# NVIDIA/semantic-segmentation

Hardware: AMD Instinct MI355X
Metric: train images/sec HRNet-OCR-MScale 1024x1024 crop (higher is better)
Workload: dtype fp16; 1 GPU; train_cityscapes_sota: HRNet-OCR-MScale two-scale train step, RMI+BCE loss, crop 1024x1024, batch 1/GPU, SGD, synthetic Cityscapes-shaped batch, random init; global_batch=1, parallelism=dp1, hipgraph=True, optimizer=ssa_sgd_momentum_step, wgrad_side_stream_flush_at=256

## Files before the change

### include/semseg_hip.h

```cpp
#ifndef SEMSEG_HIP_H
#define SEMSEG_HIP_H
#include <stddef.h>
#include <stdint.h>

#ifdef __cplusplus
extern "C" {
#endif

#define SSA_OK 0
#define SSA_EINVAL (-1)
#define SSA_EUNSUPPORTED (-2)

int ssa_version(void);
int ssa_elem_type(void);
const char* ssa_source_sha(void);

int ssa_group_begin(void);
int ssa_group_end(void* stream);
int ssa_group_abort(void);
long ssa_launch_count(int reset);

typedef struct ssa_profile_rec {
  char kernel[120];
  long launches, jobs;
  double total_us, flops, bytes;
} ssa_profile_rec;
int ssa_profile_begin(void);
int ssa_profile_note(double flops, double bytes);
int ssa_profile_end(ssa_profile_rec* out, int max_recs);

typedef struct ssa_conv_desc {
  int B, H, W, Cin;
  int ldx;
  int Ho, Wo, Cout;
  int ldy;
  int KH, KW;
  int stride, pad, dil;
  int transposed;
  int Kpad;
  int out_f32;
  int cfg;
} ssa_conv_desc;

int ssa_conv2d_igemm(const ssa_conv_desc* d, const void* x, const void* w_packed,
                     const float* bias, void* y, void* stream);

int ssa_conv2d_igemm_stats(const ssa_conv_desc* d, const void* x, const void* w_packed,
                           const float* bias, void* y, double* stats, void* stream);

int ssa_conv2d_tile_supported(const ssa_conv_desc* d);
int ssa_conv2d_tile(const ssa_conv_desc* d, const void* x, const void* w_frag,
                    const float* bias, void* y, double* stats, void* stream);
int ssa_bn_stat_replicas(void);
int ssa_conv2d_tile_aux(const ssa_conv_desc* d, const void* x, const void* w_frag,
                        const float* bias, void* y, double* stats, const void* aux, int ldaux,
                        const float* coef, int aux_mode, void* stream);

int ssa_conv2d_tile_p_supported(const ssa_conv_desc* d);
int ssa_conv_tile_strip(int units);
int ssa_conv2d_tile_p(const ssa_conv_desc* d, const void* x, const void* w_frag, const float* bias, void* y,
                      double* stats, const void* aux, int ldaux, const float* coef, int aux_mode, void* stream);

int ssa_conv2d_halo_supported(const ssa_conv_desc* d);
int ssa_conv2d_halo(const ssa_conv_desc* d, const void* x, const void* w_frag,
                    const float* bias, void* y, double* stats, void* stream);

int ssa_conv2d_gemm_wide_supported(const ssa_conv_desc* d);
int ssa_conv2d_gemm_wide(const ssa_conv_desc* d, const void* x, const void* w_frag, const float* bias,
                         void* y, double* stats, void* stream);

int ssa_conv2d_halo_reg_supported(const ssa_conv_desc* d);
int ssa_conv2d_halo_reg(const ssa_conv_desc* d, const void* x, const void* w_frag, const float* bias,
                        void* y, double* stats, void* stream);

int ssa_conv2d_halo5_supported(const ssa_conv_desc* d);
int ssa_conv2d_halo5(const ssa_conv_desc* d, const void* x, const void* w_frag, const float* bias,
                     void* y, double* stats, void* stream);

int ssa_conv2d_igemm_tile(const ssa_conv_desc* d);
int ssa_conv2d_igemm_affine(const ssa_conv_desc* d, const void* x, const void* w_packed, const float* bias, void* y,
                            const float* coef, const void* residual, int ldres, int relu, void* stream);


int ssa_conv2d_dgrad_s2(int B, int H, int W, int Cin, int lddx, int Ho, int Wo, int cout_pad,
                        int lddy, const void* dy, const void* const* w_cls, const int* kpad_cls,
                        void* dx, void* stream);

int ssa_pack_filter(const float* w_oihw, void* w_packed, int Cout, int Cin,
                    int KH, int KW, int cin_pad, int cout_pad, int Kpad,
                    int mode, void* stream);

int ssa_conv2d_wgrad_plan(const ssa_conv_desc* d, int cout_pad, int* nsplit,
                          size_t* ws_bytes);
int ssa_conv2d_wgrad(const ssa_conv_desc* d, const void* x, const void* dy,
                     int lddy, int cout_pad, int nsplit, float* partial,
                     void* stream);
int ssa_conv2d_wgrad_reduce(const float* partial, int nsplit, int cout_pad,
                            int Cout, int Cin_pad, int Cin, int KH, int KW,
                            float* dw_oihw, int accumulate, void* stream);

typedef struct ssa_pack_job {
  const float* w_oihw;
  void* w_packed;
  long elem_begin;
  int Cout, Cin, KH, KW, cin_pad, cout_pad, Kpad, mode, rows;
  int layout;
} ssa_pack_job;
int ssa_pack_filters_batched(const void* jobs_dev, int njobs, int blocks_per_job,
                             void* stream);
int ssa_pack_tile_channels(int KH, int KW);
int ssa_pack_filters_tiled(const void* jobs_dev, const void* tiles_dev, int ntiles,
                           int max_ct_taps, void* stream);

int ssa_conv2d_wgrad_tile_plan(const ssa_conv_desc* d, int cout_pad, int* nsplit,
                               size_t* ws_bytes);
int ssa_conv2d_wgrad_tile(const ssa_conv_desc* d, const void* x, const void* dy,
                          int lddy, int cout_pad, int nsplit, float* partial,
                          void* stream);
int ssa_conv2d_wgrad_tile_geometry(int Cin, int cout_pad, int* parts, int* slots, int* kind);
int ssa_conv2d_wgrad_head_plan(const ssa_conv_desc* d, int cout_pad, int* nsplit,
                               size_t* ws_bytes);
int ssa_conv2d_wgrad_head(const ssa_conv_desc* d, const void* x, const void* dy,
                          int lddy, int cout_pad, int nsplit, float* partial,
                          void* stream);

int ssa_colsum_bf16(const void* x, long P, int C, int ld, float* out,
                    double* scratch2c, void* stream);

int ssa_pad_cast_f32_bf16(const float* x, long P, int C, int ldx, void* y,
                          int Cpad, void* stream);

int ssa_bn_stats(const void* x, long P, int C, int ld, double* sums, int zero_sums,
                 void* stream);
int ssa_bn_apply_train(const void* x, int ldx, const void* residual, int ldr, void* z,
                       int ldz, long P, int C, const double* sums, int nrep, double count,
                       const float* gamma, const float* beta, float* running_mean,
                       float* running_var, long* num_batches_tracked, float momentum,
                       float eps, float* coef, float* pass_stats, int relu,
                       const float* post, long pix_per_img, void* sign_mask, void* stream);
typedef struct ssa_bn_update_job {
  float* running_mean;
  float* running_var;
  long* num_batches_tracked;
  const float* pass_stats[8];
  int C, npass;
  float momentum;
  int pad_;
} ssa_bn_update_job;
int ssa_bn_update_running_batched(const void* jobs_dev, int njobs, int max_channels,
                                  void* stream);
typedef struct ssa_bn_eval_job {
  const float* gamma;
  const float* beta;
  const float* running_mean;
  const float* running_var;
  float* coef;
  int C;
  float eps;
} ssa_bn_eval_job;
int ssa_bn_finalize_eval_batched(const void* jobs_dev, int njobs, int max_channels, void* stream);
int ssa_bn_finalize(const double* sums, double count, int C, const float* gamma,
                    const float* beta, float* running_mean, float* running_var,
                    float momentum, float eps, int use_running, float* scale,
                    float* shift, float* mean, float* invstd, void* stream);
int ssa_bn_apply(const void* x, int ldx, const void* residual, int ldr, void* z,
                 int ldz, long P, int C, const float* scale, const float* shift,
                 int relu, const float* post, long pix_per_img, void* stream);
int ssa_bn_bwd_reduce(const void* x, int ldx, const void* dz, int lddz,
                      const void* z, int ldz, long P, int C, const float* mean,
                      const float* invstd, int relu, const float* post,
                      long pix_per_img, double* sums, int nrep, int zero_sums,
                      const float* mask_scale, const float* mask_shift, const void* sign_mask, void* stream);
int ssa_bn_bwd_apply(const void* x, int ldx, const void* dz, int lddz,
                     const void* z, int ldz, void* dx, int lddx, void* dres,
                     int lddres, long P, int C, const float* gamma,
                     const float* mean, const float* invstd, const double* sums,
                     int nrep, double count, int relu, const float* post,
                     long pix_per_img, float* dgamma, float* dbeta,
                     float param_grad_scale, const float* mask_scale,
                     const float* mask_shift, int accumulate_param_grads, const void* sign_mask, void* stream);
int ssa_add_bn_stats(const void* a, int lda, const void* b, int ldb, void* s, int lds, long P,
                     int C, double* sums, int zero_sums, void* stream);
int ssa_bn_bwd_apply_add(const void* x, int ldx, const void* dz, int lddz,
                         const void* z, int ldz, void* dx, int lddx, void* dres,
                         int lddres, long P, int C, const float* gamma,
                         const float* mean, const float* invstd, const double* sums,
                         int nrep, double count, int relu, const float* post,
                         long pix_per_img, float* dgamma, float* dbeta,
                         float param_grad_scale, const float* mask_scale,
                         const float* mask_shift, int accumulate_param_grads, const void* sign_mask,
                         const void* dadd, int lddadd, void* stream);
int ssa_bn_param_grads(const double* sums, int C, float* dgamma, float* dbeta,
                       void* stream);

int ssa_p2p_buffer_bytes(int world, long slot_doubles, size_t* bytes);
int ssa_p2p_allreduce_f64(double* data, long n, void* const* peers_dev, int rank, int world,
                          unsigned long long* seq_dev, long slot_doubles, void* stream);
int ssa_p2p_timeouts(unsigned* out);
int ssa_p2p_vmm_alloc(size_t bytes, void** ptr, int* fd, size_t* mapped_bytes);
int ssa_p2p_vmm_import(int fd, size_t mapped_bytes, void** ptr);
int ssa_p2p_vmm_unmap(void* ptr, size_t mapped_bytes);

int ssa_sum_act(const void* a, const void* b, const void* c, const void* d,
                void* z, long n, int relu, void* stream);
int ssa_relu_bwd(const void* dz, const void* z, void* g, long n, void* stream);
int ssa_nchw_f32_to_nhwc_bf16(const float* x, void* y, int B, int C, int H, int W,
                              int cpad, void* stream);

int ssa_image_resize_to_nhwc_bf16(const float* x, int B, int C, int Hi, int Wi,
                                  void* y, int Ho, int Wo, int cpad, void* stream);
int ssa_image_resize_to_nhwc(const float* x, int B, int C, int Hi, int Wi,
                             void* y, int Ho, int Wo, int cpad, int align_corners, void* stream);

int ssa_bilinear_fwd(const void* x, int in_dtype, int B, int Hi, int Wi, int C,
                     int ldx, void* y, int out_dtype, int Ho, int Wo, int ldy,
                     void* stream);
int ssa_bilinear_bwd(const void* dy, int dy_dtype, int B, int Ho, int Wo, int C,
                     int lddy, void* dx, int dx_dtype, int Hi, int Wi, int lddx,
                     void* stream);
int ssa_bilinear_bwd_x(const void* dy, int dy_dtype, int B, int Ho, int Wo, int C, int lddy, float* tmp, int Wi,
                       void* stream);
int ssa_bilinear_bwd_y(const float* tmp, int B, int Ho, int Wi, int C, void* dx, int dx_dtype, int Hi, int lddx,
                       void* stream);
// ... 268 lines not shown
```

### semantic-segmentation_amd/csrc/conv_halo_reg.hip

```cpp
#include "conv_epilogue.h"
#include "group.h"
#include "../../include/semseg_hip.h"
#include <stdlib.h>
#include <type_traits>

#ifndef SSA_HREG_DRAIN
#define SSA_HREG_DRAIN (-1)
#endif

namespace {

struct HaloRegArgs {
  const bf16_t* x; const uint4* wfrag; const float* bias; bf16_t* y; double* stats;
  int ldx, Cin, ldy, B, H, W, Cout, nb_total, tiles_x, tiles_y;
};

template <int CK>
struct ConvHaloReg3 {
  typedef HaloRegArgs Args;
  static constexpr int NT = 256;
  static constexpr int WPE = 2;
  static constexpr int NB = 8, TW = 32, TH = 4, BM = TW * TH;
  static constexpr int HW_ = TW + 2, HH_ = TH + 2;
  static constexpr int CP = CK / 8;
  static constexpr int NPIECE = HH_ * HW_ * 8;
  static constexpr int IT = (NPIECE + NT - 1) / NT;
  static constexpr int HWI = (NPIECE + 63) / 64;
  static constexpr int HALO_BYTES = HWI * 1024;
  static constexpr int CST = CK / 16;
  static constexpr int TAPS = 9;
  static constexpr size_t PIPE_BYTES = 2 * (size_t)HALO_BYTES;
  static constexpr int LDC = NB * 32 + 8;
  static constexpr size_t EPI_BYTES = (size_t)BM * LDC * 2;
  static constexpr size_t LDS_BYTES = PIPE_BYTES > EPI_BYTES ? PIPE_BYTES : EPI_BYTES;
  static_assert(CK == 64 || CK == 48, "chunk width");
  static_assert(2 * LDS_BYTES <= 160 * 1024, "two workgroups per CU");

  static __device__ __forceinline__ void run(const Args& a, const int bx, const int by, const int ) {
  const uint4* __restrict__ wfrag = a.wfrag;
  const int ldx = a.ldx, Cin = a.Cin, H = a.H, W = a.W, nb_total = a.nb_total;
  const int tiles_x = a.tiles_x, tiles_y = a.tiles_y;
  SSA_DYN_LDS(unsigned char, smem);

  const int tid = threadIdx.x, lane = tid & 63;
  const int wn = __builtin_amdgcn_readfirstlane(tid >> 6);
  int bid = bx;
  const int tx_i = bid % tiles_x; bid /= tiles_x;
  const int ty_i = bid % tiles_y; bid /= tiles_y;
  const int b = bid;
  const int nb0 = by * NB;
  const int x0 = tx_i * TW, y0 = ty_i * TH;
  const int nchunk = Cin / CK;
  const int csteps = Cin / 16;
  const int ksteps = TAPS * csteps;

  const bf16_t* xb = a.x + (long)b * H * W * ldx;
  unsigned g_off[IT];
  unsigned dma_ok = 0;
#pragma unroll
  for (int i = 0; i < IT; ++i) {
    const int piece = tid + i * NT;
    const int pix = piece >> 3;
    const int hy = pix / HW_, hx = pix - hy * HW_;
    const int q = (piece & 7) ^ ((hx >> 1) & 7);
    const int iy = y0 - 1 + hy, ix = x0 - 1 + hx;
    const bool ok = piece < NPIECE && q < CP && (unsigned)iy < (unsigned)H && (unsigned)ix < (unsigned)W;
    g_off[i] = ok ? (unsigned)((((long)iy * W + ix) * ldx + q * 8) * 2) : 0u;
    dma_ok |= (ok ? 1u : 0u) << i;
  }
  const unsigned lds0 = ssa_lds_addr(smem);
  auto halo_dma = [&](int chunk, int buf) {
    const bf16_t* src = xb + chunk * CK;
#pragma unroll
    for (int i = 0; i < IT; ++i) {
      if ((dma_ok >> i) & 1u) ssa_glds16_untracked_m0(src, g_off[i], lds0 + buf * HALO_BYTES + (i * 4 + wn) * 1024);
    }
  };

  for (int o = tid * 16; o < 2 * HALO_BYTES; o += NT * 16) *reinterpret_cast<uint4*>(smem + o) = make_uint4(0, 0, 0, 0);
  __syncthreads();

  const unsigned char* wq[2];
#pragma unroll
  for (int ni = 0; ni < 2; ++ni) {
    const int nbg = min(nb0 + wn * 2 + ni, nb_total - 1);
    wq[ni] = reinterpret_cast<const unsigned char*>(wfrag + (long)nbg * ksteps * 64);
  }
  const unsigned lane16 = lane * 16;
  constexpr int R = CST == 4 ? 6 : 3;
  constexpr int ROWK = 3 * CST;
  static_assert(ROWK % R == 0 && R <= ROWK, "ring period");
  bf16x8_t bq[R][2];
  auto load_b = [&](const int slot, const int kstep) {
#pragma unroll
    for (int ni = 0; ni < 2; ++ni)
      bq[slot][ni] = *reinterpret_cast<const bf16x8_t*>(wq[ni] + (long)kstep * 1024 + lane16);
  };

  const int a_col = lane & 31;
  const int a_half = (lane >> 5) << 4;
  f32x16_t acc[4][2];
#pragma unroll
  for (int mi = 0; mi < 4; ++mi)
#pragma unroll
    for (int ni = 0; ni < 2; ++ni)
#pragma unroll
      for (int r = 0; r < 16; ++r) acc[mi][ni][r] = 0.f;

  bf16x8_t af[4];
  int a_base[3];
#pragma unroll
  for (int kw = 0; kw < 3; ++kw) {
    const int hx = a_col + kw;
    a_base[kw] = (hx << 7) | ((((hx >> 1) & 7) << 4) ^ a_half);
  }
  auto rd1 = [&](const unsigned char* Hrow, const int kw, const int j, const int mi) {
    af[mi] = *reinterpret_cast<const bf16x8_t*>(Hrow + mi * (HW_ * 128) + (a_base[kw] ^ (j << 5)));
  };

  halo_dma(0, 0);
#pragma unroll
  for (int q = 0; q < R; ++q) load_b(q, (q / CST) * csteps + q % CST);
  ssa_wait_vm_barrier<0, 0>();
  for (int c = 0; c < nchunk; ++c) {
    const unsigned char* Hc = smem + (c & 1) * HALO_BYTES;
    if (c + 1 < nchunk) halo_dma(c + 1, (c + 1) & 1);
#pragma unroll
    for (int mi = 0; mi < 4; ++mi) rd1(Hc, 0, 0, mi);
#pragma nounroll
    for (int kh = 0; kh < 3; ++kh) {
      const unsigned char* Hrow = Hc + kh * (HW_ * 128);
      const int krow = kh * 3 * csteps + c * CST;
      const int krow_n = kh < 2 ? krow + 3 * csteps : min(c + 1, nchunk - 1) * CST;
#pragma unroll
      for (int kw = 0; kw < 3; ++kw) {
#pragma unroll
        for (int j = 0; j < CST; ++j) {
          const int pos = kw * CST + j, slot = pos % R;
#pragma unroll
          for (int mi = 0; mi < 4; ++mi) {
#pragma unroll
            for (int ni = 0; ni < 2; ++ni) acc[mi][ni] = ssa_mfma32(af[mi], bq[slot][ni], acc[mi][ni]);
            if (j + 1 < CST) rd1(Hrow, kw, j + 1, mi);
            else if (kw < 2) rd1(Hrow, kw + 1, 0, mi);
            else rd1(Hrow + HW_ * 128, 0, 0, mi);
          }
          const int pn = pos + R;
          if (pn < ROWK) load_b(slot, krow + (pn / CST) * csteps + pn % CST);
          else load_b(slot, krow_n + ((pn - ROWK) / CST) * csteps + (pn - ROWK) % CST);
#ifndef SSA_EMU
          __builtin_amdgcn_sched_group_barrier(0x008, 2, 0);
          __builtin_amdgcn_sched_group_barrier(0x020, 2, 0);
          __builtin_amdgcn_sched_group_barrier(0x100, 1, 0);
          __builtin_amdgcn_sched_group_barrier(0x008, 2, 0);
          __builtin_amdgcn_sched_group_barrier(0x100, 1, 0);
          __builtin_amdgcn_sched_group_barrier(0x008, 2, 0);
          __builtin_amdgcn_sched_group_barrier(0x100, 1, 0);
          __builtin_amdgcn_sched_group_barrier(0x008, 2, 0);
          __builtin_amdgcn_sched_group_barrier(0x100, 1, 0);
          __builtin_amdgcn_sched_barrier(0);
#endif
        }
      }
    }
    ssa_wait_vm_barrier<SSA_HREG_DRAIN < 0 ? 2 * R : SSA_HREG_DRAIN, 0>();
  }

  const float* __restrict__ bias = a.bias;
  double* __restrict__ stats = a.stats;
  const int ldy = a.ldy, Cout = a.Cout;
  bf16_t* Cs = reinterpret_cast<bf16_t*>(smem);
  double* st = stats ? stats + (long)(bx % ssa::kStatReplicas) * 2 * Cout : nullptr;
  ssa::epi_stage<LDC>(acc, bias, stats != nullptr, 0, wn * 64, nb0 * 32, Cout, Cs, lane,
                      [&](int row) { return y0 + row / TW < H && x0 + row % TW < W; },
                      [&](int, int n, float sv, float qv) {
                        if (n < Cout) {
                          atomicAdd(&st[n], (double)sv);
                          atomicAdd(&st[Cout + n], (double)qv);
                        }
                      });
  __syncthreads();
  bf16_t* yb = a.y + (long)b * H * W * ldy;
  ssa::epi_store_rows<BM, NB * 32, NT>(Cs, nb0 * 32, Cout, tid, [&](int row, bf16_t*& p) {
    const int oy = y0 + row / TW, ox = x0 + row % TW;
    p = yb + ((long)oy * W + ox) * ldy;
    return oy < H && ox < W;
  });
  }
};

bool reg_shape_ok(const ssa_conv_desc* d) {
  if (!d || d->KH != 3 || d->KW != 3 || d->stride != 1 || d->dil != 1 || d->transposed || d->pad != 1) return false;
  if (d->Ho != d->H || d->Wo != d->W || d->out_f32) return false;
  if (d->ldx % 8 || d->Cout % 8 || d->ldy % 8 || ssa::pick_ck(d->Cin) == 0) return false;
  return (long)d->H * d->W * d->ldx * 2 < (1L << 32);
}

}

extern "C" {

int ssa_conv2d_halo_reg_supported(const ssa_conv_desc* d) { return reg_shape_ok(d) ? 1 : 0; }

int ssa_conv2d_halo_reg(const ssa_conv_desc* dp, const void* x, const void* w_frag, const float* bias,
                        void* y, double* stats, void* stream) {
  if (!dp || !x || !w_frag || !y) return SSA_EINVAL;
  if (!reg_shape_ok(dp)) return SSA_EUNSUPPORTED;
  if (!ssa::conv_ptrs_ok(x, y, w_frag)) return SSA_EINVAL;
  const ssa_conv_desc& d = *dp;
  HaloRegArgs a;
  a.x = (const bf16_t*)x; a.wfrag = (const uint4*)w_frag; a.bias = bias; a.y = (bf16_t*)y; a.stats = stats;
  a.ldx = d.ldx; a.Cin = d.Cin; a.ldy = d.ldy; a.B = d.B; a.H = d.H; a.W = d.W; a.Cout = d.Cout;
  a.nb_total = (d.Cout + 31) / 32;
  a.tiles_x = (d.W + 31) / 32; a.tiles_y = (d.H + 3) / 4;
  const int gx = a.tiles_x * a.tiles_y * d.B, gy = (a.nb_total + 7) / 8;
  if (ssa::pick_ck(d.Cin) == 64) {
    typedef ConvHaloReg3<64> K;
    return ssa::submit<K>(a, gx, gy, K::LDS_BYTES, (hipStream_t)stream);
  }
  typedef ConvHaloReg3<48> K;
  return ssa::submit<K>(a, gx, gy, K::LDS_BYTES, (hipStream_t)stream);
}

}
```

### semantic-segmentation_amd/csrc/group.h

```cpp
#pragma once
#include <hip/hip_runtime.h>
#include <string.h>
#include <type_traits>
#include <vector>

namespace ssa {

constexpr int kKernargBudget = 3840;

template <class K, class = void> struct MaxJobs { static constexpr int value = 16; };
template <class K> struct MaxJobs<K, std::void_t<decltype(K::MAXJOBS)>> { static constexpr int value = K::MAXJOBS; };

template <class K>
struct GroupLimits {
  static constexpr int per_job = (int)sizeof(typename K::Args) + 8;
  static constexpr int raw = (kKernargBudget - 16) / per_job;
  static constexpr int cap = MaxJobs<K>::value;
  static constexpr int jobs = raw > cap ? cap : (raw < 1 ? 1 : raw);
};

template <class K>
struct GroupTable {
  int n, pad_;
  int end[GroupLimits<K>::jobs];
  int gx[GroupLimits<K>::jobs];
  typename K::Args a[GroupLimits<K>::jobs];
};

template <class K, class = void> struct WavesPerEu { static constexpr int value = 1; };
template <class K> struct WavesPerEu<K, std::void_t<decltype(K::WPE)>> { static constexpr int value = K::WPE; };

template <class K>
__global__ __launch_bounds__(K::NT, WavesPerEu<K>::value) void k_single(const typename K::Args a) {
  K::run(a, blockIdx.x, blockIdx.y, gridDim.x);
}

template <class K>
__global__ __launch_bounds__(K::NT, WavesPerEu<K>::value) void k_grouped(const GroupTable<K> t) {
  constexpr int J = GroupLimits<K>::jobs;
  const int bx = (int)blockIdx.x;
  int j = 0;
#pragma unroll
  for (int i = 0; i + 1 < J; ++i) j += bx >= t.end[i] ? 1 : 0;
  const int prev = t.end[j > 0 ? j - 1 : 0];
  const int gx = t.gx[j];
  const int v = bx - (j > 0 ? prev : 0);
  int vx = v, vy = 0;
  if (v >= gx) { vy = v / gx; vx = v - vy * gx; }
  K::run(t.a[j], vx, vy, gx);
}

struct Bucket {
  const void* key;
  int (*flush)(Bucket&, hipStream_t);
  std::vector<unsigned char> args;
  std::vector<int> gx, gy;
  std::vector<double> flops, bytes;
  size_t lds;
};

bool profiling();
void profile_take_note(double* flops, double* bytes);
void* profile_open(const char* kernel, hipStream_t s);
void profile_close(void* h, hipStream_t s, int jobs, double flops, double bytes);

template <class K>
const char* kernel_name() { return __PRETTY_FUNCTION__; }

struct GroupState {
  int depth = 0;
  int error = 0;
  std::vector<Bucket> buckets;
};

GroupState& group_state();
void count_launches(int n);


constexpr int kMaxDevices = 16;
struct LdsLimit { size_t set_to[kMaxDevices] = {}; };

inline int raise_lds_limit(const void* fn, size_t lds, size_t threshold, LdsLimit* lim) {
  if (lds <= threshold) return 0;
  int dev = 0;
  if (hipGetDevice(&dev) != hipSuccess || dev < 0 || dev >= kMaxDevices) dev = 0;
  if (lds > lim->set_to[dev]) {
    hipError_t e = hipFuncSetAttribute(fn, hipFuncAttributeMaxDynamicSharedMemorySize, (int)lds);
    if (e != hipSuccess) return (int)e;
    lim->set_to[dev] = lds;
  }
  return 0;
}

template <class K>
int ensure_lds(const void* fn, size_t lds, LdsLimit* lim) {
  return raise_lds_limit(fn, lds, 64 * 1024, lim);
}

template <class K>
int flush_bucket(Bucket& b, hipStream_t s) {
  typedef typename K::Args Args;
  constexpr int J = GroupLimits<K>::jobs;
  static LdsLimit lds_single, lds_grouped;
  const int n = (int)b.gx.size();
  for (int j0 = 0; j0 < n; j0 += J) {
    const int cnt = n - j0 < J ? n - j0 : J;
    if (cnt == 1) {
      Args a;
      memcpy(&a, b.args.data() + (size_t)j0 * sizeof(Args), sizeof(Args));
      if (int e = ensure_lds<K>((const void*)k_single<K>, b.lds, &lds_single)) return e;
      void* ph = profiling() ? profile_open(kernel_name<K>(), s) : nullptr;
      hipLaunchKernelGGL(k_single<K>, dim3(b.gx[j0], b.gy[j0]), dim3(K::NT), b.lds, s, a);
      if (ph) profile_close(ph, s, 1, b.flops[j0], b.bytes[j0]);
    } else {
      GroupTable<K> t;
      memset(&t, 0, sizeof(t));
      t.n = cnt;
      int total = 0;
      for (int i = 0; i < cnt; ++i) {
        total += b.gx[j0 + i] * b.gy[j0 + i];
        t.end[i] = total;
        t.gx[i] = b.gx[j0 + i];
        memcpy(&t.a[i], b.args.data() + (size_t)(j0 + i) * sizeof(Args), sizeof(Args));
      }
      for (int i = cnt - 1; i < J; ++i) t.end[i] = 0x7fffffff;
      if (int e = ensure_lds<K>((const void*)k_grouped<K>, b.lds, &lds_grouped)) return e;
      void* ph = profiling() ? profile_open(kernel_name<K>(), s) : nullptr;
      hipLaunchKernelGGL(k_grouped<K>, dim3(total), dim3(K::NT), b.lds, s, t);
      if (ph) {
        double fl = 0, by = 0;
        for (int i = 0; i < cnt; ++i) { fl += b.flops[j0 + i]; by += b.bytes[j0 + i]; }
        profile_close(ph, s, cnt, fl, by);
      }
    }
    count_launches(1);
    hipError_t e = hipGetLastError();
    if (e != hipSuccess) return (int)e;
  }
  return 0;
}

template <class K>
int submit(const typename K::Args& a, int gx, int gy, size_t lds, hipStream_t s) {
  typedef typename K::Args Args;
  static_assert(sizeof(GroupTable<K>) <= kKernargBudget + 64, "job table exceeds the kernel-argument budget");
  if (gx <= 0 || gy <= 0) return -1;
  GroupState& g = group_state();
  double note_f = 0, note_b = 0;
  const bool prof = profiling();
  if (prof) profile_take_note(&note_f, &note_b);
  if (g.depth == 0) {
    static LdsLimit lds_single;
    if (int e = ensure_lds<K>((const void*)k_single<K>, lds, &lds_single)) return e;
    void* ph = prof ? profile_open(kernel_name<K>(), s) : nullptr;
    hipLaunchKernelGGL(k_single<K>, dim3(gx, gy), dim3(K::NT), lds, s, a);
    if (ph) profile_close(ph, s, 1, note_f, note_b);
    count_launches(1);
    hipError_t e = hipGetLastError();
    return e == hipSuccess ? 0 : (int)e;
  }
  const void* key = (const void*)k_grouped<K>;
  Bucket* b = nullptr;
  for (Bucket& c : g.buckets)
    if (c.key == key) { b = &c; break; }
  if (!b) {
    g.buckets.push_back(Bucket{key, &flush_bucket<K>, {}, {}, {}, {}, {}, 0});
    b = &g.buckets.back();
  }
  const size_t off = b->args.size();
  b->args.resize(off + sizeof(Args));
  memcpy(b->args.data() + off, &a, sizeof(Args));
  b->gx.push_back(gx);
  b->gy.push_back(gy);
  b->flops.push_back(note_f);
  b->bytes.push_back(note_b);
  if (lds > b->lds) b->lds = lds;
  return 0;
}

}
```

### semantic-segmentation_amd/semseg_amd/_lib.py

```python
import ctypes
import os
from ctypes import c_int, c_long, c_float, c_double, c_void_p, c_size_t, c_uint64, POINTER

_HERE = os.path.dirname(os.path.abspath(__file__))
ACT = os.environ.get("SSA_ACT_DTYPE", "bf16").lower()
if ACT in ("f16", "float16", "half"):
    ACT = "fp16"
if ACT not in ("bf16", "fp16"):
    raise RuntimeError("SSA_ACT_DTYPE must be bf16 or fp16, not %r" % ACT)
LIB_PATH = os.path.normpath(os.path.join(_HERE, "..", "lib", "libsemseg_hip.so" if ACT == "bf16" else "libsemseg_hip_f16.so"))
CSRC = os.path.normpath(os.path.join(_HERE, "..", "csrc"))

_LIB = None


def source_sha():
    import glob
    import hashlib
    files = sorted(glob.glob(os.path.join(CSRC, "*.hip"))) + sorted(glob.glob(os.path.join(CSRC, "*.h"))) + [
        os.path.normpath(os.path.join(_HERE, "..", "..", "include", "semseg_hip.h"))]
    if not files or not all(os.path.exists(f) for f in files):
        return None
    h = hashlib.sha256()
    for f in files:
        with open(f, "rb") as fh:
            h.update(fh.read())
    return h.hexdigest()[:16]


class PackJob(ctypes.Structure):
    _fields_ = [("w", c_void_p), ("out", c_void_p), ("elem_begin", c_long)] + [(n, c_int) for n in (
        "Cout", "Cin", "KH", "KW", "cin_pad", "cout_pad", "Kpad", "mode", "rows", "layout")]


class BnEvalJob(ctypes.Structure):
    _fields_ = [("gamma", c_void_p), ("beta", c_void_p), ("running_mean", c_void_p), ("running_var", c_void_p),
                ("coef", c_void_p), ("C", c_int), ("eps", c_float)]


class BnUpdateJob(ctypes.Structure):
    _fields_ = [("running_mean", c_void_p), ("running_var", c_void_p), ("num_batches_tracked", c_void_p),
                ("pass_stats", c_void_p * 8), ("C", c_int), ("npass", c_int), ("momentum", c_float),
                ("pad_", c_int)]


class ProfileRec(ctypes.Structure):
    _fields_ = [("kernel", ctypes.c_char * 120), ("launches", c_long), ("jobs", c_long),
                ("total_us", c_double), ("flops", c_double), ("bytes", c_double)]


class ConvDesc(ctypes.Structure):
    _fields_ = [(n, c_int) for n in (
        "B", "H", "W", "Cin", "ldx", "Ho", "Wo", "Cout", "ldy", "KH", "KW",
        "stride", "pad", "dil", "transposed", "Kpad", "out_f32", "cfg")]


class DwConvDesc(ctypes.Structure):
    _fields_ = [(n, c_int) for n in ("B", "H", "W", "C", "ldx", "Ho", "Wo", "ldy", "stride", "dil")]


class GConvDesc(ctypes.Structure):
    _fields_ = [(n, c_int) for n in ("B", "H", "W", "C", "G", "ldx", "Ho", "Wo", "ldy", "stride", "dil")]


class JitterProgram(ctypes.Structure):
    _fields_ = [("n_ops", c_int), ("op", c_int * 4), ("factor", c_float * 3), ("hue_byte", c_int)]


class GblurTaps(ctypes.Structure):
    _fields_ = [("radius", c_int), ("w", c_double * 6)]


class RandaugProgram(ctypes.Structure):
    _fields_ = [("n_ops", c_int), ("op", c_int * 8), ("value", c_double * 8), ("matrix", (c_double * 6) * 8)]


_P = c_void_p
_SIGS = {
    "ssa_version": ([], c_int),
    "ssa_elem_type": ([], c_int),
    "ssa_source_sha": ([], ctypes.c_char_p),
    "ssa_group_begin": ([], c_int),
    "ssa_group_end": ([_P], c_int),
    "ssa_group_abort": ([], c_int),
    "ssa_launch_count": ([c_int], c_long),
    "ssa_profile_begin": ([], c_int),
    "ssa_profile_note": ([c_double, c_double], c_int),
    "ssa_profile_end": ([POINTER(ProfileRec), c_int], c_int),
    "ssa_conv2d_igemm": ([POINTER(ConvDesc), _P, _P, _P, _P, _P], c_int),
    "ssa_conv2d_igemm_stats": ([POINTER(ConvDesc), _P, _P, _P, _P, _P, _P], c_int),
    "ssa_conv2d_igemm_tile": ([POINTER(ConvDesc)], c_int),
    "ssa_conv2d_tile_supported": ([POINTER(ConvDesc)], c_int),
    "ssa_conv2d_tile": ([POINTER(ConvDesc), _P, _P, _P, _P, _P, _P], c_int),
    "ssa_conv2d_tile_aux": ([POINTER(ConvDesc), _P, _P, _P, _P, _P, _P, c_int, _P, c_int, _P], c_int),
    "ssa_bn_stat_replicas": ([], c_int),
    "ssa_conv2d_tile_p_supported": ([POINTER(ConvDesc)], c_int),
    "ssa_conv_tile_strip": ([c_int], c_int),
    "ssa_conv2d_tile_p": ([POINTER(ConvDesc), _P, _P, _P, _P, _P, _P, c_int, _P, c_int, _P], c_int),
    "ssa_conv2d_halo_supported": ([POINTER(ConvDesc)], c_int),
    "ssa_conv2d_halo": ([POINTER(ConvDesc), _P, _P, _P, _P, _P, _P], c_int),
    "ssa_conv2d_gemm_wide_supported": ([POINTER(ConvDesc)], c_int),
    "ssa_conv2d_gemm_wide": ([POINTER(ConvDesc), _P, _P, _P, _P, _P, _P], c_int),
    "ssa_conv2d_halo_reg_supported": ([POINTER(ConvDesc)], c_int),
    "ssa_conv2d_halo_reg": ([POINTER(ConvDesc), _P, _P, _P, _P, _P, _P], c_int),
    "ssa_conv2d_halo5_supported": ([POINTER(ConvDesc)], c_int),
    "ssa_conv2d_halo5": ([POINTER(ConvDesc), _P, _P, _P, _P, _P, _P], c_int),
    "ssa_pack_filter": ([_P, _P] + [c_int] * 8 + [_P], c_int),
    "ssa_conv2d_wgrad_plan": ([POINTER(ConvDesc), c_int, POINTER(c_int), POINTER(c_size_t)], c_int),
    "ssa_conv2d_wgrad": ([POINTER(ConvDesc), _P, _P, c_int, c_int, c_int, _P, _P], c_int),
    "ssa_conv2d_wgrad_tile_plan": ([POINTER(ConvDesc), c_int, POINTER(c_int), POINTER(c_size_t)], c_int),
    "ssa_conv2d_wgrad_tile": ([POINTER(ConvDesc), _P, _P, c_int, c_int, c_int, _P, _P], c_int),
    "ssa_conv2d_wgrad_tile_geometry": ([c_int, c_int, POINTER(c_int), POINTER(c_int), POINTER(c_int)], c_int),
    "ssa_conv2d_wgrad_head_plan": ([POINTER(ConvDesc), c_int, POINTER(c_int), POINTER(c_size_t)], c_int),
    "ssa_conv2d_wgrad_head": ([POINTER(ConvDesc), _P, _P, c_int, c_int, c_int, _P, _P], c_int),
    "ssa_conv2d_wgrad_reduce": ([_P] + [c_int] * 7 + [_P, c_int, _P], c_int),
    "ssa_colsum_bf16": ([_P, c_long, c_int, c_int, _P, _P, _P], c_int),
    "ssa_pad_cast_f32_bf16": ([_P, c_long, c_int, c_int, _P, c_int, _P], c_int),
    "ssa_bn_stats": ([_P, c_long, c_int, c_int, _P, c_int, _P], c_int),
    "ssa_bn_apply_train": ([_P, c_int, _P, c_int, _P, c_int, c_long, c_int, _P, c_int, c_double, _P, _P, _P, _P,
                            _P, c_float, c_float, _P, _P, c_int, _P, c_long, _P, _P], c_int),
    "ssa_bn_update_running_batched": ([_P, c_int, c_int, _P], c_int),
    "ssa_pack_filters_batched": ([_P, c_int, c_int, _P], c_int),
    "ssa_pack_tile_channels": ([c_int, c_int], c_int),
    "ssa_conv2d_dgrad_s2": ([c_int] * 9 + [_P, _P, _P, _P, _P], c_int),
    "ssa_pack_filters_tiled": ([_P, _P, c_int, c_int, _P], c_int),
    "ssa_conv2d_igemm_affine": ([POINTER(ConvDesc), _P, _P, _P, _P, _P, _P, c_int, c_int, _P], c_int),
    "ssa_bn_finalize_eval_batched": ([_P, c_int, c_int, _P], c_int),
    "ssa_bn_finalize": ([_P, c_double, c_int, _P, _P, _P, _P, c_float, c_float, c_int,
                         _P, _P, _P, _P, _P], c_int),
    "ssa_bn_apply": ([_P, c_int, _P, c_int, _P, c_int, c_long, c_int, _P, _P, c_int, _P,
                      c_long, _P], c_int),
    "ssa_bn_bwd_reduce": ([_P, c_int, _P, c_int, _P, c_int, c_long, c_int, _P, _P, c_int, _P,
                           c_long, _P, c_int, c_int, _P, _P, _P, _P], c_int),
    "ssa_bn_bwd_apply": ([_P, c_int, _P, c_int, _P, c_int, _P, c_int, _P, c_int, c_long, c_int,
                          _P, _P, _P, _P, c_int, c_double, c_int, _P, c_long, _P, _P, c_float, _P, _P, c_int, _P, _P], c_int),
    "ssa_add_bn_stats": ([_P, c_int, _P, c_int, _P, c_int, c_long, c_int, _P, c_int, _P], c_int),
    "ssa_bn_bwd_apply_add": ([_P, c_int, _P, c_int, _P, c_int, _P, c_int, _P, c_int, c_long, c_int,
                              _P, _P, _P, _P, c_int, c_double, c_int, _P, c_long, _P, _P, c_float, _P, _P, c_int, _P,
                              _P, c_int, _P], c_int),
    "ssa_bn_param_grads": ([_P, c_int, _P, _P, _P], c_int),
    "ssa_p2p_buffer_bytes": ([c_int, c_long, POINTER(c_size_t)], c_int),
    "ssa_p2p_allreduce_f64": ([_P, c_long, _P, c_int, c_int, _P, c_long, _P], c_int),
    "ssa_p2p_timeouts": ([_P], c_int),
    "ssa_p2p_vmm_alloc": ([c_size_t, POINTER(c_void_p), POINTER(c_int), POINTER(c_size_t)], c_int),
    "ssa_p2p_vmm_import": ([c_int, c_size_t, POINTER(c_void_p)], c_int),
    "ssa_p2p_vmm_unmap": ([_P, c_size_t], c_int),
    "ssa_sum_act": ([_P, _P, _P, _P, _P, c_long, c_int, _P], c_int),
    "ssa_relu_bwd": ([_P, _P, _P, c_long, _P], c_int),
    "ssa_nchw_f32_to_nhwc_bf16": ([_P, _P, c_int, c_int, c_int, c_int, c_int, _P], c_int),
    "ssa_image_resize_to_nhwc_bf16": ([_P, c_int, c_int, c_int, c_int, _P, c_int, c_int, c_int, _P], c_int),
    "ssa_bilinear_fwd": ([_P, c_int, c_int, c_int, c_int, c_int, c_int, _P, c_int, c_int, c_int,
                          c_int, _P], c_int),
    "ssa_bilinear_bwd": ([_P, c_int, c_int, c_int, c_int, c_int, c_int, _P, c_int, c_int, c_int,
                          c_int, _P], c_int),
    "ssa_bilinear_bwd_x": ([_P, c_int, c_int, c_int, c_int, c_int, c_int, _P, c_int, _P], c_int),
    "ssa_bilinear_bwd_y": ([_P, c_int, c_int, c_int, c_int, _P, c_int, c_int, c_int, _P], c_int),
    "ssa_image_resize_to_nhwc": ([_P, c_int, c_int, c_int, c_int, _P, c_int, c_int, c_int, c_int, _P], c_int),
    "ssa_resize_bilinear_fwd": ([_P, c_int, c_int, c_int, c_int, c_int, c_int, _P, c_int, c_int, c_int,
                                 c_int, c_int, _P], c_int),
    "ssa_resize_bilinear_bwd": ([_P, c_int, c_int, c_int, c_int, c_int, c_int, _P, c_int, c_int, c_int,
                                 c_int, c_int, _P], c_int),
    "ssa_resize_bilinear_bwd_x": ([_P, c_int, c_int, c_int, c_int, c_int, c_int, _P, c_int, c_int, _P], c_int),
    "ssa_resize_bilinear_bwd_y": ([_P, c_int, c_int, c_int, c_int, _P, c_int, c_int, c_int, c_int, _P], c_int),
    "ssa_maxpool3x3s2_fwd": ([_P, c_int, c_int, c_int, c_int, c_int, _P, _P, c_int, c_int, _P], c_int),
    "ssa_maxpool3x3s2_bwd": ([_P, _P, c_int, c_int, c_int, c_int, _P, c_int, c_int, _P], c_int),
    "ssa_maxpool3x3s2c_fwd": ([_P, c_int, c_int, c_int, c_int, c_int, _P, _P, c_int, c_int, _P], c_int),
    "ssa_maxpool3x3s2c_bwd": ([_P, _P, c_int, c_int, c_int, c_int, _P, c_int, c_int, _P], c_int),
    "ssa_gconv3x3": ([POINTER(GConvDesc), _P, _P, _P, _P, _P], c_int),
    "ssa_gconv3x3_bwd_plan": ([POINTER(GConvDesc), POINTER(c_size_t)], c_int),
    "ssa_gconv3x3_bwd": ([POINTER(GConvDesc), _P, _P, c_int, _P, _P, c_int, _P, c_int, _P, _P], c_int),
    "ssa_se_plan": ([c_int, c_long, c_int, c_int, POINTER(c_size_t)], c_int),
    "ssa_se_squeeze_gate": ([_P, c_int, c_int, c_long, c_int, c_int, _P, _P, _P, _P, _P, _P, _P, _P, _P], c_int),
    "ssa_se_apply": ([_P, c_int, _P, c_int, _P, _P, c_int, c_int, c_long, c_int, c_int, _P], c_int),
    "ssa_se_bwd_reduce": ([_P, c_int, _P, c_int, _P, c_int, c_int, c_long, c_int, c_int, _P, _P, _P], c_int),
    "ssa_se_gate_bwd": ([_P, _P, _P, _P, _P, _P, c_int, c_long, c_int, c_int, _P, _P, _P, _P, _P, c_int, _P, _P], c_int),
    "ssa_se_apply_bwd": ([_P, c_int, _P, c_int, _P, _P, c_int, c_long, c_int, c_int, _P, c_int, _P, c_int, _P], c_int),
    "ssa_dwconv3x3": ([POINTER(DwConvDesc), _P, _P, _P, _P, _P, c_int, _P], c_int),
    "ssa_dwconv3x3_bwd_plan": ([POINTER(DwConvDesc), POINTER(c_size_t)], c_int),
    "ssa_dwconv3x3_bwd": ([POINTER(DwConvDesc), _P, _P, c_int, _P, _P, c_int, _P, c_int, _P, _P], c_int),
    "ssa_global_avg_pool_fwd": ([_P, c_int, c_int, c_long, c_int, _P, _P], c_int),
    "ssa_global_avg_pool_bwd": ([_P, c_int, c_long, c_int, _P, _P], c_int),
    "ssa_resize_nearest_u8": ([_P, c_int, c_int, c_int, _P, c_int, c_int, _P, _P, _P], c_int),
    "ssa_softmax_hw_stats": ([_P, c_int, c_long, c_int, _P, _P], c_int),
    "ssa_softmax_hw_probs": ([_P, c_int, c_long, c_int, _P, _P, c_int, _P], c_int),
    "ssa_rowdot_f32": ([_P, _P, c_int, c_int, _P, _P], c_int),
    "ssa_softmax_hw_bwd": ([_P, c_int, c_long, c_int, _P, _P, c_int, _P, _P, c_int, c_int, _P], c_int),
    "ssa_softmax_lastdim_fwd": ([_P, c_int, c_long, c_int, c_float, _P, c_int, _P], c_int),
    "ssa_softmax_lastdim_bwd": ([_P, c_int, c_long, c_int, c_float, _P, c_int, _P, c_int, _P], c_int),
    "ssa_pack_matrix": ([_P, c_int, c_int, c_int, c_int, c_int, _P, c_int, c_int, _P], c_int),
    "ssa_ocr_attn_supported": ([c_int, c_int], c_int),
    "ssa_ocr_attn_fwd": ([_P, c_int, _P, _P, c_long, c_int, c_int, c_float, _P, c_int, _P], c_int),
    "ssa_ocr_attn_bwd": ([_P, c_int, _P, _P, _P, c_int, c_long, c_int, c_int, c_float, _P, c_int, _P, _P, _P], c_int),
    "ssa_sigmoid_fwd": ([_P, _P, c_long, _P], c_int),
    "ssa_sigmoid_bwd": ([_P, _P, _P, c_long, _P], c_int),
    "ssa_bcast_mul_fwd": ([_P, _P, _P, c_long, c_int, _P], c_int),
    "ssa_bcast_mul_bwd": ([_P, _P, _P, _P, _P, c_long, c_int, _P], c_int),
    "ssa_attn_blend_fwd": ([_P, _P, _P, _P, c_long, c_int, _P], c_int),
    "ssa_attn_blend_bwd": ([_P, _P, _P, _P, _P, c_long, c_int, c_int, _P], c_int),
    "ssa_ce_fwd": ([_P, c_int, _P, c_long, c_int, c_int, _P, _P, _P], c_int),
    "ssa_bce_fwd": ([_P, c_int, _P, c_long, c_int, _P, _P, _P], c_int),
    "ssa_loss_finalize": ([_P, c_double, _P, _P], c_int),
    "ssa_bce_bwd": ([_P, c_int, _P, c_long, c_int, _P, c_double, _P, c_double, _P, _P], c_int),
    "ssa_scale_grad": ([_P, c_long, _P, c_double, _P, c_double, _P], c_int),
    "ssa_scale_grad_to": ([_P, _P, c_long, _P, c_double, _P, c_double, _P], c_int),
    "ssa_rmi_pool": ([_P, c_int, _P, c_int, c_int, c_int, c_int, _P, _P, c_int, c_int, _P], c_int),
    "ssa_rmi_gram": ([_P, _P, c_int, c_int, c_int, _P, _P], c_int),
    "ssa_rmi_solve": ([_P, c_int, c_int, c_int, _P, _P, _P], c_int),
    "ssa_rmi_finalize": ([_P, c_int, c_int, _P, _P], c_int),
    "ssa_rmi_bwd_pooled": ([_P, _P, _P, c_int, c_int, c_int, _P, _P], c_int),
    "ssa_rmi_bwd_logits": ([_P, c_int, _P, c_int, c_int, c_int, c_int, _P, c_int, c_int, _P,
                            c_double, _P, c_int, _P], c_int),
    "ssa_rmi_bwd_logits_bce": ([_P, c_int, _P, c_int, c_int, c_int, c_int, _P, c_int, c_int, _P, c_double, _P, c_double, _P,
                                c_double, _P, _P], c_int),
    "ssa_relax_mask_labels": ([_P, c_int, c_int, c_int, c_int, c_int, c_int, c_int, c_uint64, c_uint64, _P, _P, _P], c_int),
    "ssa_relax_mask_multihot": ([_P, c_int, c_int, c_int, c_int, _P, _P, _P], c_int),
    "ssa_relax_multihot": ([_P, c_int, c_int, c_int, c_int, _P, _P], c_int),
    "ssa_relax_weights": ([_P, c_int, c_int, c_double, c_int, _P, _P, _P], c_int),
    "ssa_relax_nll_fwd": ([_P, c_int, _P, _P, c_int, c_int, c_int, c_int, _P, _P], c_int),
    "ssa_relax_nll_finalize": ([_P, _P, c_int, c_int, c_int, c_int, _P, _P], c_int),
    "ssa_relax_nll_bwd": ([_P, c_int, _P, _P, _P, c_int, c_int, c_int, c_int, _P, _P, _P], c_int),
    "ssa_image_u8_crop_flip_normalize": ([_P, c_int, c_int, c_int, c_int, c_int, c_int, c_int, _P, _P, _P, c_int, _P],
                                         c_int),
    "ssa_resample_u8": ([_P, c_int, c_int, c_int, c_int, _P, c_int, _P, _P, c_int, _P], c_int),
    "ssa_label_u8_crop_flip": ([_P, c_int, c_int, c_int, c_int, c_int, c_int, c_int, _P, _P], c_int),
    "ssa_jitter_luma_sum": ([_P, c_int, c_int, c_int, c_int, c_int, c_int, POINTER(JitterProgram), _P, _P], c_int),
    "ssa_jitter_apply_u8": ([_P, c_int, c_int, c_int, c_int, c_int, c_int, c_int, POINTER(JitterProgram), _P, _P, _P],
                            c_int),
    "ssa_jitter_crop_flip_normalize": ([_P, c_int, c_int, c_int, c_int, c_int, c_int, c_int, POINTER(JitterProgram), _P,
                                        _P, _P, _P, c_int, _P], c_int),
    "ssa_gblur_u8": ([_P, c_int, c_int, c_int, c_int, c_int, c_int, c_int, POINTER(JitterProgram), _P, POINTER(GblurTaps),
                      _P, _P, _P], c_int),
    "ssa_gblur_crop_flip_normalize": ([_P, c_int, c_int, c_int, c_int, c_int, c_int, c_int, POINTER(JitterProgram), _P,
                                       POINTER(GblurTaps), _P, _P, _P, _P, c_int, _P], c_int),
    "ssa_randaug_u8": ([_P, _P, c_int, c_int, c_int, c_int, c_int, c_int, c_int, POINTER(RandaugProgram), c_int, _P, _P, _P,
                        _P, _P, _P], c_int),
    "ssa_class_centroids_u8": ([_P, c_int, c_int, c_int, c_int, c_int, c_int, _P, _P, _P, _P], c_int),
    "ssa_pad_u8": ([_P, c_int, c_int, c_int, c_int, c_int, c_int, c_int, ctypes.c_char_p, _P, _P], c_int),
    "ssa_autolabel_u8": ([_P, _P, _P, c_int, c_int, c_int, c_int, c_int, c_int, ctypes.c_char_p, c_int, c_int, c_int, c_int,
                          c_int, c_int, c_int, c_int, _P, _P, _P, c_int, _P], c_int),
    "ssa_confusion_matrix": ([_P, c_int, _P, c_long, c_int, _P, _P, _P], c_int),
    "ssa_eval_tail": ([_P, _P, c_int, c_int, c_int, c_int, c_int, c_int, _P, c_int, c_float, c_float, _P, _P, _P, _P, _P,
                       _P, _P], c_int),
    "ssa_dump_tail": ([_P, c_long, POINTER(c_float), POINTER(c_float), _P, _P, _P, _P, _P, _P, c_float, c_int, c_int,
                       _P, _P, _P, _P, _P, _P, _P, _P], c_int),
    "ssa_mask_u8": ([_P, c_long, _P, _P], c_int),
    "ssa_sgd_momentum_step": ([_P, _P, _P, _P, c_int, c_float, _P, c_float, c_float, c_int, _P, _P], c_int),
    "ssa_amp_check_grads": ([_P, _P, c_int, _P, _P], c_int),
    "ssa_amp_update": ([_P, c_int, c_float, c_float, c_float, c_float, _P], c_int),
    "ssa_amp_update_counted": ([_P, _P, c_int, c_float, c_float, c_float, c_float, _P], c_int),
    "ssa_adam_advance": ([_P, c_int, c_int, c_double, c_double, _P, _P], c_int),
    "ssa_adam_step": ([_P, _P, _P, _P, _P, _P, _P, c_int, c_int, c_float, _P, c_double, c_double, c_float, c_float,
                       _P, _P], c_int),
    "ssa_ewise_f32": ([c_int, _P, _P, _P, c_long, _P], c_int),
    "ssa_ewise_bwd_f32": ([c_int, _P, _P, _P, _P, _P, c_long, _P], c_int),
    "ssa_axpy_f32": ([_P, c_float, _P, c_long, c_int, _P], c_int),
# ... 50 lines not shown
```

Before: 53.82 images/s.

## Split tail-wave tiles into half-height tiles in halo_reg conv to balance waves

Adds a host-side plan step that counts total workgroups against the CU count and, when the last wave is only partly filled and a cost model favours it, splits the trailing tiles into two half-height (2-row) tiles. The kernel body is templated on the row count so half tiles use fewer MFMA accumulators and a smaller halo, and the epilogue stats are merged across the two accumulator halves. The goal is to shorten the tail-wave imbalance (wave quantization) in 3x3 conv launches. The risks are extra halo-load overhead for the split tiles and a more complex epilogue stats path.

```diff
diff --git a/include/semseg_hip.h b/include/semseg_hip.h
--- a/include/semseg_hip.h
+++ b/include/semseg_hip.h
@@ -69,6 +69,7 @@
 int ssa_conv2d_gemm_wide(const ssa_conv_desc* d, const void* x, const void* w_frag, const float* bias,
                          void* y, double* stats, void* stream);
 
+int ssa_conv_halo_reg_slots(int slots);
 int ssa_conv2d_halo_reg_supported(const ssa_conv_desc* d);
 int ssa_conv2d_halo_reg(const ssa_conv_desc* d, const void* x, const void* w_frag, const float* bias,
                         void* y, double* stats, void* stream);
diff --git a/semantic-segmentation_amd/csrc/conv_halo_reg.hip b/semantic-segmentation_amd/csrc/conv_halo_reg.hip
--- a/semantic-segmentation_amd/csrc/conv_halo_reg.hip
+++ b/semantic-segmentation_amd/csrc/conv_halo_reg.hip
@@ -13,20 +13,58 @@
 struct HaloRegArgs {
   const bf16_t* x; const uint4* wfrag; const float* bias; bf16_t* y; double* stats;
   int ldx, Cin, ldy, B, H, W, Cout, nb_total, tiles_x, tiles_y;
+  int split_from, ntiles;
 };
+
+constexpr double kHalfTileCost = 0.58;
+int g_slots = -1;
+
+int device_slots() {
+  static int cached[ssa::kMaxDevices] = {};
+  int dev = 0;
+  if (hipGetDevice(&dev) != hipSuccess || dev < 0 || dev >= ssa::kMaxDevices) dev = 0;
+  if (cached[dev] == 0) {
+    int cus = 0;
+    if (hipDeviceGetAttribute(&cus, hipDeviceAttributeMultiprocessorCount, dev) != hipSuccess || cus <= 0) return 0;
+    cached[dev] = cus;
+  }
+  return cached[dev];
+}
+
+int split_count(long N, int S) {
+  if (S <= 0 || N <= 0) return 0;
+  const long r = N % S;
+  if (r == 0) return 0;
+  const long short_rounds = (2 * r + S - 1) / S;
+  return short_rounds * kHalfTileCost < 1.0 ? (int)r : 0;
+}
+
+void plan_jobs(HaloRegArgs* a, int* gx, int* gy, int n) {
+  long N = 0;
+  for (int j = 0; j < n; ++j) N += (long)gx[j] * gy[j];
+  int left = split_count(N, g_slots < 0 ? device_slots() : g_slots);
+  for (int j = n - 1; j >= 0 && left > 0; --j) {
+    const int nj = gx[j] * gy[j];
+    const int take = left < nj ? left : nj;
+    a[j].split_from = nj - take;
+    gx[j] = nj + take;
+    gy[j] = 1;
+    left -= take;
+  }
+}
 
 template <int CK>
 struct ConvHaloReg3 {
   typedef HaloRegArgs Args;
+  static void plan(Args* a, int* gx, int* gy, int n) { plan_jobs(a, gx, gy, n); }
   static constexpr int NT = 256;
   static constexpr int WPE = 2;
   static constexpr int NB = 8, TW = 32, TH = 4, BM = TW * TH;
   static constexpr int HW_ = TW + 2, HH_ = TH + 2;
   static constexpr int CP = CK / 8;
-  static constexpr int NPIECE = HH_ * HW_ * 8;
-  static constexpr int IT = (NPIECE + NT - 1) / NT;
-  static constexpr int HWI = (NPIECE + 63) / 64;
-  static constexpr int HALO_BYTES = HWI * 1024;
+  static constexpr int npiece(int MR) { return (MR + 2) * HW_ * 8; }
+  static constexpr int halo_bytes(int MR) { return (npiece(MR) + 63) / 64 * 1024; }
+  static constexpr int HALO_BYTES = halo_bytes(TH);
   static constexpr int CST = CK / 16;
   static constexpr int TAPS = 9;
   static constexpr size_t PIPE_BYTES = 2 * (size_t)HALO_BYTES;
@@ -37,6 +75,20 @@
   static_assert(2 * LDS_BYTES <= 160 * 1024, "two workgroups per CU");
 
   static __device__ __forceinline__ void run(const Args& a, const int bx, const int by, const int ) {
+    if (a.split_from < 0) { body<TH>(a, bx, by, 0); return; }
+    const int h = bx - a.split_from;
+    const int u = h < 0 ? bx : a.split_from + (h >> 1);
+    const int slice = u / a.ntiles, tile = u - slice * a.ntiles;
+    if (h < 0) body<TH>(a, tile, slice, 0);
+    else body<TH / 2>(a, tile, slice, (h & 1) * (TH / 2));
+  }
+
+  template <int MR>
+  static __device__ __forceinline__ void body(const Args& a, const int bx, const int by, const int yoff) {
+  constexpr int NPIECE = npiece(MR);
+  constexpr int IT = (NPIECE + NT - 1) / NT;
+  constexpr int HALO_BYTES = halo_bytes(MR);
+  constexpr int BM = MR * TW;
   const uint4* __restrict__ wfrag = a.wfrag;
   const int ldx = a.ldx, Cin = a.Cin, H = a.H, W = a.W, nb_total = a.nb_total;
   const int tiles_x = a.tiles_x, tiles_y = a.tiles_y;
@@ -49,7 +101,9 @@
   const int ty_i = bid % tiles_y; bid /= tiles_y;
   const int b = bid;
   const int nb0 = by * NB;
-  const int x0 = tx_i * TW, y0 = ty_i * TH;
+  const int x0 = tx_i * TW, y0 = ty_i * TH + yoff;
+  if constexpr (MR != TH)
+    if (y0 >= a.H) return;
   const int nchunk = Cin / CK;
   const int csteps = Cin / 16;
   const int ksteps = TAPS * csteps;
@@ -99,15 +153,15 @@
 
   const int a_col = lane & 31;
   const int a_half = (lane >> 5) << 4;
-  f32x16_t acc[4][2];
-#pragma unroll
-  for (int mi = 0; mi < 4; ++mi)
+  f32x16_t acc[MR / 2][2][2];
+#pragma unroll
+  for (int mi = 0; mi < MR; ++mi)
 #pragma unroll
     for (int ni = 0; ni < 2; ++ni)
 #pragma unroll
-      for (int r = 0; r < 16; ++r) acc[mi][ni][r] = 0.f;
-
-  bf16x8_t af[4];
+      for (int r = 0; r < 16; ++r) acc[mi >> 1][mi & 1][ni][r] = 0.f;
+
+  bf16x8_t af[MR];
   int a_base[3];
 #pragma unroll
   for (int kw = 0; kw < 3; ++kw) {
@@ -126,7 +180,7 @@
     const unsigned char* Hc = smem + (c & 1) * HALO_BYTES;
     if (c + 1 < nchunk) halo_dma(c + 1, (c + 1) & 1);
 #pragma unroll
-    for (int mi = 0; mi < 4; ++mi) rd1(Hc, 0, 0, mi);
+    for (int mi = 0; mi < MR; ++mi) rd1(Hc, 0, 0, mi);
 #pragma nounroll
     for (int kh = 0; kh < 3; ++kh) {
       const unsigned char* Hrow = Hc + kh * (HW_ * 128);
@@ -138,9 +192,9 @@
         for (int j = 0; j < CST; ++j) {
           const int pos = kw * CST + j, slot = pos % R;
 #pragma unroll
-          for (int mi = 0; mi < 4; ++mi) {
-#pragma unroll
-            for (int ni = 0; ni < 2; ++ni) acc[mi][ni] = ssa_mfma32(af[mi], bq[slot][ni], acc[mi][ni]);
+          for (int mi = 0; mi < MR; ++mi) {
+#pragma unroll
+            for (int ni = 0; ni < 2; ++ni) acc[mi >> 1][mi & 1][ni] = ssa_mfma32(af[mi], bq[slot][ni], acc[mi >> 1][mi & 1][ni]);
             if (j + 1 < CST) rd1(Hrow, kw, j + 1, mi);
             else if (kw < 2) rd1(Hrow, kw + 1, 0, mi);
             else rd1(Hrow + HW_ * 128, 0, 0, mi);
@@ -154,10 +208,12 @@
           __builtin_amdgcn_sched_group_barrier(0x100, 1, 0);
           __builtin_amdgcn_sched_group_barrier(0x008, 2, 0);
           __builtin_amdgcn_sched_group_barrier(0x100, 1, 0);
-          __builtin_amdgcn_sched_group_barrier(0x008, 2, 0);
-          __builtin_amdgcn_sched_group_barrier(0x100, 1, 0);
-          __builtin_amdgcn_sched_group_barrier(0x008, 2, 0);
-          __builtin_amdgcn_sched_group_barrier(0x100, 1, 0);
+          if constexpr (MR == 4) {
+            __builtin_amdgcn_sched_group_barrier(0x008, 2, 0);
+            __builtin_amdgcn_sched_group_barrier(0x100, 1, 0);
+            __builtin_amdgcn_sched_group_barrier(0x008, 2, 0);
+            __builtin_amdgcn_sched_group_barrier(0x100, 1, 0);
+          }
           __builtin_amdgcn_sched_barrier(0);
 #endif
         }
@@ -171,12 +227,21 @@
   const int ldy = a.ldy, Cout = a.Cout;
   bf16_t* Cs = reinterpret_cast<bf16_t*>(smem);
   double* st = stats ? stats + (long)(bx % ssa::kStatReplicas) * 2 * Cout : nullptr;
-  ssa::epi_stage<LDC>(acc, bias, stats != nullptr, 0, wn * 64, nb0 * 32, Cout, Cs, lane,
-                      [&](int row) { return y0 + row / TW < H && x0 + row % TW < W; },
-                      [&](int, int n, float sv, float qv) {
+  auto valid = [&](int row) { return y0 + row / TW < H && x0 + row % TW < W; };
+  double ups[2] = {0., 0.}, upq[2] = {0., 0.};
+  if constexpr (MR == TH)
+    ssa::epi_stage<LDC>(acc[0], bias, stats != nullptr, 0, wn * 64, nb0 * 32, Cout, Cs, lane, valid,
+                        [&](int col, int, float sv, float qv) {
+                          const bool second = col - wn * 64 >= 32;
+                          if (second) { ups[1] = (double)sv; upq[1] = (double)qv; }
+                          else { ups[0] = (double)sv; upq[0] = (double)qv; }
+                        });
+  ssa::epi_stage<LDC>(acc[MR / 2 - 1], bias, stats != nullptr, BM - 2 * TW, wn * 64, nb0 * 32, Cout, Cs, lane, valid,
+                      [&](int col, int n, float sv, float qv) {
                         if (n < Cout) {
-                          atomicAdd(&st[n], (double)sv);
-                          atomicAdd(&st[Cout + n], (double)qv);
+                          const bool second = col - wn * 64 >= 32;
+                          atomicAdd(&st[n], (second ? ups[1] : ups[0]) + (double)sv);
+                          atomicAdd(&st[Cout + n], (second ? upq[1] : upq[0]) + (double)qv);
                         }
                       });
   __syncthreads();
@@ -201,6 +266,12 @@
 extern "C" {
 
 int ssa_conv2d_halo_reg_supported(const ssa_conv_desc* d) { return reg_shape_ok(d) ? 1 : 0; }
+
+int ssa_conv_halo_reg_slots(int slots) {
+  const int prev = g_slots;
+  g_slots = slots < 0 ? -1 : slots;
+  return prev;
+}
 
 int ssa_conv2d_halo_reg(const ssa_conv_desc* dp, const void* x, const void* w_frag, const float* bias,
                         void* y, double* stats, void* stream) {
@@ -214,6 +285,7 @@
   a.nb_total = (d.Cout + 31) / 32;
   a.tiles_x = (d.W + 31) / 32; a.tiles_y = (d.H + 3) / 4;
   const int gx = a.tiles_x * a.tiles_y * d.B, gy = (a.nb_total + 7) / 8;
+  a.split_from = -1; a.ntiles = gx;
   if (ssa::pick_ck(d.Cin) == 64) {
     typedef ConvHaloReg3<64> K;
     return ssa::submit<K>(a, gx, gy, K::LDS_BYTES, (hipStream_t)stream);
diff --git a/semantic-segmentation_amd/csrc/group.h b/semantic-segmentation_amd/csrc/group.h
--- a/semantic-segmentation_amd/csrc/group.h
+++ b/semantic-segmentation_amd/csrc/group.h
@@ -29,6 +29,10 @@
 
 template <class K, class = void> struct WavesPerEu { static constexpr int value = 1; };
 template <class K> struct WavesPerEu<K, std::void_t<decltype(K::WPE)>> { static constexpr int value = K::WPE; };
+
+template <class K, class = void> struct HasPlan : std::false_type {};
+template <class K>
+struct HasPlan<K, std::void_t<decltype(K::plan((typename K::Args*)nullptr, (int*)nullptr, (int*)nullptr, 0))>> : std::true_type {};
 
 template <class K>
 __global__ __launch_bounds__(K::NT, WavesPerEu<K>::value) void k_single(const typename K::Args a) {
@@ -105,6 +109,12 @@
   const int n = (int)b.gx.size();
   for (int j0 = 0; j0 < n; j0 += J) {
     const int cnt = n - j0 < J ? n - j0 : J;
+    if constexpr (HasPlan<K>::value) {
+      Args pa[J];
+      memcpy(pa, b.args.data() + (size_t)j0 * sizeof(Args), (size_t)cnt * sizeof(Args));
+      K::plan(pa, b.gx.data() + j0, b.gy.data() + j0, cnt);
+      memcpy(b.args.data() + (size_t)j0 * sizeof(Args), pa, (size_t)cnt * sizeof(Args));
+    }
     if (cnt == 1) {
       Args a;
       memcpy(&a, b.args.data() + (size_t)j0 * sizeof(Args), sizeof(Args));
@@ -152,8 +162,15 @@
   if (g.depth == 0) {
     static LdsLimit lds_single;
     if (int e = ensure_lds<K>((const void*)k_single<K>, lds, &lds_single)) return e;
+    const Args* la = &a;
+    [[maybe_unused]] Args planned;
+    if constexpr (HasPlan<K>::value) {
+      planned = a;
+      K::plan(&planned, &gx, &gy, 1);
+      la = &planned;
+    }
     void* ph = prof ? profile_open(kernel_name<K>(), s) : nullptr;
-    hipLaunchKernelGGL(k_single<K>, dim3(gx, gy), dim3(K::NT), lds, s, a);
+    hipLaunchKernelGGL(k_single<K>, dim3(gx, gy), dim3(K::NT), lds, s, *la);
     if (ph) profile_close(ph, s, 1, note_f, note_b);
     count_launches(1);
     hipError_t e = hipGetLastError();
diff --git a/semantic-segmentation_amd/semseg_amd/_lib.py b/semantic-segmentation_amd/semseg_amd/_lib.py
--- a/semantic-segmentation_amd/semseg_amd/_lib.py
+++ b/semantic-segmentation_amd/semseg_amd/_lib.py
@@ -101,6 +101,7 @@
     "ssa_conv2d_halo": ([POINTER(ConvDesc), _P, _P, _P, _P, _P, _P], c_int),
     "ssa_conv2d_gemm_wide_supported": ([POINTER(ConvDesc)], c_int),
     "ssa_conv2d_gemm_wide": ([POINTER(ConvDesc), _P, _P, _P, _P, _P, _P], c_int),
+    "ssa_conv_halo_reg_slots": ([c_int], c_int),
     "ssa_conv2d_halo_reg_supported": ([POINTER(ConvDesc)], c_int),
     "ssa_conv2d_halo_reg": ([POINTER(ConvDesc), _P, _P, _P, _P, _P, _P], c_int),
     "ssa_conv2d_halo5_supported": ([POINTER(ConvDesc)], c_int),
```

Measured after the change: 53.30 images/s. Within noise of the previous version (-1.0%).
